# SIMPLE-BuildingSimulation/heat

Measured on AMD Instinct MI355X. Metric: surface-node-updates/sec, higher is better.
Workload: dtype f64

## Files before the change

heat_amd/csrc/batch.hip:

```cpp
#include <hip/hip_runtime.h>
#include <rccl/rccl.h>

#include <dlfcn.h>

#include <algorithm>
#include <cmath>
#include <cstdarg>
#include <cstdio>
#include <cstdlib>
#include <cstring>
#include <limits>
#include <mutex>
#include <numeric>
#include <string>
#include <vector>

#include "../../include/heat_amd.h"
#include "kernels.hpp"
#include "layout.hpp"
#include "hostpool.hpp"
#include "plan.hpp"

using namespace heat;

// ... 55 lines not shown
        r.CommDestroy = reinterpret_cast<decltype(r.CommDestroy)>(dlsym(h, "ncclCommDestroy"));
        r.AllGather = reinterpret_cast<decltype(r.AllGather)>(dlsym(h, "ncclAllGather"));
        r.AllReduce = reinterpret_cast<decltype(r.AllReduce)>(dlsym(h, "ncclAllReduce"));
        r.GetErrorString = reinterpret_cast<decltype(r.GetErrorString)>(dlsym(h, "ncclGetErrorString"));
        if (!r.GetUniqueId || !r.CommInitRank || !r.CommDestroy || !r.AllGather || !r.AllReduce || !r.GetErrorString) {
            st.err = "symbols missing";
            dlclose(h);
            return;
        }
        st.err.clear();
        r.handle = h;
    });
    return st.r.handle ? &st.r : nullptr;
}

#define RCCL_TRY(R, expr)                                                                             \
    do {                                                                                              \
        ncclResult_t e_ = (expr);                                                                     \
        if (e_ != ncclSuccess)                                                                        \
            return fail(HEAT_E_COMM, "%s failed: %s (%s:%d)", #expr, (R)->GetErrorString(e_), __FILE__, __LINE__); \
    } while (0)

template <typename T>
struct DevBuf {
    T *p = nullptr;
    size_t n = 0;
    ~DevBuf() { release(); }
    void release() {
        if (p) (void)hipFree(p);
        p = nullptr;
        n = 0;
    }
    hipError_t alloc(size_t count) {
        release();
        n = count;
        if (count == 0) return hipSuccess;
        return hipMalloc(reinterpret_cast<void **>(&p), count * sizeof(T));
    }
    hipError_t upload(const std::vector<T> &h) {
        hipError_t e = alloc(h.size());
        if (e != hipSuccess || h.empty()) return e;
        return hipMemcpy(p, h.data(), h.size() * sizeof(T), hipMemcpyHostToDevice);
    }
    hipError_t zeros(size_t count) {
        hipError_t e = alloc(count);
        if (e != hipSuccess || count == 0) return e;
        e = hipMemset(p, 0, count * sizeof(T));
        if (e != hipSuccess) return e;
        return hipStreamSynchronize(nullptr);
    }
};

static const int kFusedMinSubsteps = getenv("HEAT_AMD_FUSED_MIN") ? atoi(getenv("HEAT_AMD_FUSED_MIN")) : 2;

}

struct heat_batch {
    int device = 0;
    int n_cu = 256;
    hipStream_t stream = nullptr;
    bool own_stream = false;
    static constexpr int kSideStreams = 3;
    hipStream_t side[kSideStreams] = {nullptr, nullptr, nullptr};
    hipStream_t fused_stream = nullptr;
    hipEvent_t ev_fork = nullptr, ev_join[kSideStreams] = {nullptr, nullptr, nullptr};
    int n_ranks = 1, rank = 0;
    bool use_graph = false;

    int64_t n_surf = 0, n_zones = 0, n_state = 0, n_nodes = 0, n_cav = 0;
    double dt = 0;
    int64_t algorithmic_bytes = 0;
    int64_t class_counts[5] = {0, 0, 0, 0, 0};
    int64_t n_palette = 0;

    int64_t n_fused_surfaces = 0;
    int n_stream_tiles[kNumFast] = {};
    std::vector<FusedBlock> h_fblocks[kNumFast][4];
    DevBuf<FusedBlock> d_fblocks[kNumFast][4];
    std::vector<FusedBlock> h_team_blocks[kNumFast], h_team_blocks0[kNumFast];
    std::vector<FusedSuper> h_team_supers[kNumFast];
    DevBuf<FusedBlock> d_team_blocks[kNumFast];
    DevBuf<FusedSuper> d_team_supers[kNumFast];
    DevBuf<uint32_t> d_team_zinfo;
    DevBuf<unsigned long long> d_xbuf;
    int xbuf_teams = 0;
    uint32_t team_epoch = 0;
    bool any_teams = false;
    DevBuf<unsigned int> d_fqueue;
    DevBuf<int32_t> d_fzones, d_fzone_eoff;
    DevBuf<uint16_t> d_fslots;
    DevBuf<double> d_side_area;
    DevBuf<int16_t> d_side_lzone;
    std::vector<FastTile> h_tiles0[kNumFast];
    std::vector<FusedBlock> h_fblocks0[kNumFast][4];
    int n_stream_tiles0[kNumFast] = {};
    std::vector<int32_t> h_fzones;
    DevBuf<int32_t> d_zlist_stream;
    int n_touched_stream = 0;
    std::vector<int32_t> h_zone_block;
    DevBuf<int32_t> d_stream_zones;
    int n_stream_zones = 0;
    bool any_fused = false;
    hipEvent_t ev_fused = nullptr;
    hipEvent_t ev_staged = nullptr;
    bool staged = false;
    int n_fast_tiles[kNumFast] = {};
    DevBuf<FastTile> d_fast_tiles[kNumFast];
    std::vector<FastTile> h_tiles_cur[kNumFast];
    DevBuf<FastTile> d_ulist[2];
    int n_ulist[2] = {0, 0};
    int ulist_part[2][kStreamVariants][2] = {};
    bool capturing = false;
    bool host_zones_stale = false;
    unsigned int sweep_parity = 0;
    unsigned int fused_parity = 0;
    bool class_has_chunks[kNumFast] = {};
    bool in_ulist[2][kNumFast] = {};
    bool small_in_ulist[2] = {false, false};
    bool smallcav_in_ulist[2] = {false, false};
    DevBuf<unsigned long long> d_ucount;
    size_t ucount_stride = 0;
    int n_gen_tiles = 0;
    int n_small_tiles = 0;
    int n_small_plain_tiles = 0;
    int n_smallcav_stream_tiles = 0;
    int n_smallcav_stream_tiles0 = 0;
    std::vector<GeneralTile> h_gen_tiles0;
    std::vector<GeneralTile> h_gen_tiles_cur;
    size_t nm_count_base[kNumFast + 1] = {};
    DevBuf<GeneralTile> d_gen_tiles;
    int64_t gen_base = 0;
    int64_t node_slots = 0;

    DevBuf<double> d_T, d_V, d_U, d_alpha_f, d_alpha_b, d_mass, d_scratch;
    DevBuf<int32_t> d_cav_idx;
    DevBuf<int32_t> d_cavref;
    DevBuf<uint8_t> d_cls;
    DevBuf<double> d_pal;
    DevBuf<CavityDev> d_cavs;

    DevBuf<int32_t> d_meta;
// ... 563 lines not shown
    for (int c = 0; c < kNumFast; c++) {
        const int n_super = (int)b->h_team_supers[c].size();
        if (n_super == 0) continue;
        if (n_sub > 4095) return fail(HEAT_E_INVALID_ARG, "a march call of %d sub-timesteps: the team exchange tags 4095 at most", n_sub);
        static const int team_room_env = getenv("HEAT_AMD_TEAM_ROOM") ? atoi(getenv("HEAT_AMD_TEAM_ROOM")) : 0;
        TeamShape &ts = shape[c];
        ts.room = team_room_env > 0 ? team_room_env : b->n_cu * std::min(2, fused_team_blocks_per_cu(kFastM[c], kFastNM[c], b->na.pal_stride));
        ts.team_size = 2;
        for (const FusedSuper &su : b->h_team_supers[c]) ts.team_size = std::max(ts.team_size, (int)su.n_members);
        ts.n_teams = std::min(n_super, std::max(0, ts.room - ts.room / 8) / ts.team_size);
        if (ts.n_teams >= 1 && (n_super + ts.n_teams - 1) / ts.n_teams > 1023)
            return fail(HEAT_E_SIZE, "%d clusters for %d teams: the exchange tags 1023 rounds per launch at most", n_super, ts.n_teams);
        if (ts.n_teams < 1) return fail(HEAT_E_DEVICE, "the device holds %d workgroups of the team variant: not one team", ts.room);
    }
    return HEAT_OK;
}

int enqueue_fused(heat_batch *b, int n_sub, hipStream_t st, bool streamed_beside = false) {
    TeamShape team_shape[kNumFast];
    {
        const int rc = team_shapes(b, n_sub, team_shape);
        if (rc) return rc;
    }
    FusedArgs fa{};
    {
        static const bool zigzag_off = getenv("HEAT_AMD_NO_ZIGZAG") != nullptr;
        fa.reverse = (!zigzag_off && (b->fused_parity++ & 1)) ? 1 : 0;
    }
    fa.zones = b->d_fzones.p;
    fa.zone_eoff = b->d_fzone_eoff.p;
    fa.slots = b->d_fslots.p;
    fa.side_area = b->d_side_area.p;
    fa.side_lzone = b->d_side_lzone.p;
    fa.a0 = b->d_zone_a0.p;
    fa.b0 = b->d_zone_b0.p;
    fa.vol = b->d_zone_vol.p;
    fa.zone_T = b->d_zone_T.p;
    fa.dt = b->dt;
    fa.n_sub = n_sub;
    fa.gen_tiles = b->d_gen_tiles.p;
    fa.gen_base = b->gen_base;
    fa.small_iters = b->d_nomass_iters.p + b->nm_count_base[kNumFast];
    static const int reserve_env = getenv("HEAT_AMD_FUSED_RESERVE") ? atoi(getenv("HEAT_AMD_FUSED_RESERVE")) : -1;
    const bool beside_exchange = (b->comm != nullptr && b->shared_set && b->n_shared > 0) || reserve_env >= 0 || streamed_beside;
    double streamed_share = 0.0;
    if (streamed_beside) {
        double ns = 4.0 * kWave * (b->n_gen_tiles - (b->n_small_tiles - b->n_small_plain_tiles - b->n_smallcav_stream_tiles)), nf = 0.0;
        for (int c = 0; c < kNumFast; c++) {
            ns += (double)b->n_stream_tiles[c] * kFastM[c] * kWave;
            nf += (double)(b->n_fast_tiles[c] - b->n_stream_tiles[c]) * kFastM[c] * kWave;
        }
        streamed_share = ns / std::max(ns + nf, 1.0);
    }
    const int n_cu = b->n_cu;
    if (beside_exchange && b->d_fqueue.n == 0) HIP_TRY(b->d_fqueue.zeros(kNumFast * 4));
    for (int c = 0; c < kNumFast; c++)
        for (int g2 = 0; g2 < 4; g2++) {
            const int nb = (int)b->h_fblocks[c][g2].size();
            if (nb == 0) continue;
            fa.blocks = b->d_fblocks[c][g2].p;
            fa.n_blocks = nb;
            fa.queue = nullptr;
            int grid = nb;
            if (beside_exchange) {
                const int fw = (g2 & 1) ? 8 : 4;
                static const int room_env = getenv("HEAT_AMD_FUSED_ROOM") ? atoi(getenv("HEAT_AMD_FUSED_ROOM")) : 0;
                const int room = room_env > 0 ? room_env : n_cu * fused_blocks_per_cu(kFastM[c], kFastCAV[c], g2 >> 1, fw, b->na.pal_stride);
                const int reserve = reserve_env >= 0 ? reserve_env
                                                     : std::min(room / 2, std::max(fw == 4 ? 16 : 8, (int)(room * streamed_share)));
                if (nb > room - reserve) {
                    grid = std::max(1, room - reserve);
                    fa.queue = b->d_fqueue.p + c * 4 + g2;
                    HIP_TRY(hipMemsetAsync(fa.queue, 0, sizeof(unsigned int), st));
                }
            }
            static const bool trace = getenv("HEAT_AMD_TRACE") != nullptr;
            if (trace)
                fprintf(stderr, "heat_amd: fused launch%s: %d workgroups for %d blocks (class %d, list %d, %d sub-timesteps)\n",
                        fa.queue ? " on the work queue" : "", grid, nb, c, g2, n_sub);
            b->n_fused_launches++;
            const int nm_variant = kFastNM[c] ? ((b->class_has_chunks[c] && !(g2 >> 1) && !kFastCAV[c] && kFastM[c] <= 8) ? 2 : 1) : 0;
            HIP_TRY(launch_surfaces_fused(kFastM[c], nm_variant, kFastCAV[c], g2 >> 1, (g2 & 1) ? 8 : 4, grid, b->d_fast_tiles[c].p, b->n_fast_tiles[c],
                                          b->na, b->sa, b->d_weather.p, b->d_flags.p,
                                          b->d_nomass_iters.p + b->nm_count_base[c], fa, st));
        }
    for (int c = 0; c < kNumFast; c++) {
        const int n_super = (int)b->h_team_supers[c].size();
        if (n_super == 0) continue;
        const int team_size = team_shape[c].team_size, n_teams = team_shape[c].n_teams;
        if (b->xbuf_teams < n_teams) {
            HIP_TRY(b->d_xbuf.zeros((size_t)n_teams * 2 * kTeamZones * kTeamMax * 4));
            b->xbuf_teams = n_teams;
        }
        b->team_epoch++;
        if ((b->team_epoch & 1023u) == 0) {
            HIP_TRY(hipMemsetAsync(b->d_xbuf.p, 0, b->d_xbuf.n * sizeof(unsigned long long), st));
            b->team_epoch++;
        }
        fa.blocks = b->d_team_blocks[c].p;
        fa.n_blocks = (int)b->h_team_blocks[c].size();
        fa.queue = nullptr;
        fa.supers = b->d_team_supers[c].p;
        fa.n_super = n_super;
        fa.team_zinfo = b->d_team_zinfo.p;
        fa.xbuf = b->d_xbuf.p;
        fa.tag_base = (b->team_epoch & 1023u) << 22;
        fa.team_size = team_size;
        static const bool trace = getenv("HEAT_AMD_TRACE") != nullptr;
        if (trace)
            fprintf(stderr, "heat_amd: team launch: %d teams of %d workgroups for %d clusters (class %d, %d sub-timesteps)\n",
                    n_teams, team_size, n_super, c, n_sub);
        b->n_fused_launches++;
        HIP_TRY(launch_surfaces_fused(kFastM[c], kFastNM[c], 0, 2, 4, n_teams * team_size, b->d_fast_tiles[c].p, b->n_fast_tiles[c], b->na,
                                      b->sa, b->d_weather.p, b->d_flags.p, b->d_nomass_iters.p + b->nm_count_base[c], fa, st));
    }
    return HEAT_OK;
}

hipEvent_t next_event(heat_batch *b) {
    if (b->ev_used == b->ev_pool.size()) {
        hipEvent_t e;
        if (hipEventCreate(&e) != hipSuccess) return nullptr;
        b->ev_pool.push_back(e);
    }
    return b->ev_pool[b->ev_used++];
}

struct MarchGuard {
    heat_batch *b;
    double *saved_partial;
    bool forked = false, joined = false;
    explicit MarchGuard(heat_batch *b_) : b(b_), saved_partial(b_->partial_ptr) {}
    ~MarchGuard() {
        b->partial_ptr = saved_partial;
        if (forked && !joined && b->fused_stream) (void)hipStreamSynchronize(b->fused_stream);
    }
};
// ... 2102 lines not shown
```

heat_amd/csrc/kernels.hip:

```cpp
#include <hip/hip_runtime.h>

#include <algorithm>
#include <atomic>
#include <cstdlib>

#include "device_math.hpp"
#include "kernels.hpp"
#include "layout.hpp"

namespace heat {

__device__ __forceinline__ void eval_side(const SideConst &c, const StepWeather &w, double air_t, double rad_alt,
                                          double rad_out, double surf_t, double &hs, double &rad_t, int &bad) {
    const double natural = tarp_natural(air_t, surf_t, c.cos_eff, bad);
    if ((c.kind_n & 3) == KIND_OUTDOOR) {
        const bool windward = (c.kind_n & 4) ? true : ((c.nx * w.sin_wd + c.ny * w.cos_wd) > 0.0);
        const double wf = windward ? 1.0 : 0.5;
        hs = wf * (c.forced * w.sqrt_ws) + natural;
        rad_t = rad_out;
    } else {
        hs = natural;
        rad_t = rad_alt;
    }
}
// ... 353 lines not shown
        l.zvol[threadIdx.x] = fa.vol[z];
    }
    const int n_e = fa.zone_eoff[blk.first_zone + blk.n_zones] - e_first;
    for (int e = threadIdx.x; e < n_e; e += n_threads) l.slots[fa.slots[e_first + e]] = (unsigned short)e;
    __syncthreads();
}

struct FusedPre {
    int e_first, n_e, zoff, z, slot0;
    double zT, za0, zb0, zvol;
};
__device__ __forceinline__ void fused_pre_a(const FusedBlock &blk, const FusedArgs &fa, FusedPre &p) {
    p = FusedPre{0, 0, 0, 0, 0, 0.0, 0.0, 0.0, 0.0};
    const int nz = blk.n_zones;
    if (nz > 0) {
        p.e_first = fa.zone_eoff[blk.first_zone];
        p.n_e = fa.zone_eoff[blk.first_zone + nz];
        p.zoff = fa.zone_eoff[blk.first_zone + min((int)threadIdx.x, nz)];
        p.z = fa.zones[blk.first_zone + min((int)threadIdx.x, nz - 1)];
    }
}
__device__ __forceinline__ void fused_pre_b(const FusedBlock &blk, const FusedArgs &fa, FusedPre &p) {
    if (blk.n_zones > 0) {
        p.n_e -= p.e_first;
        p.zoff -= p.e_first;
        p.zT = fa.zone_T[p.z];
        p.za0 = fa.a0[p.z];
        p.zb0 = fa.b0[p.z];
        p.zvol = fa.vol[p.z];
        if (p.n_e > 0) p.slot0 = fa.slots[p.e_first + min((int)threadIdx.x, p.n_e - 1)];
    }
}
__device__ __forceinline__ void fused_block_init(const FusedBlock &blk, const FusedArgs &fa, const FusedLds &l, int n_threads,
                                                 const FusedPre &p) {
    if ((int)threadIdx.x <= blk.n_zones) l.zoff[threadIdx.x] = p.zoff;
    if ((int)threadIdx.x < blk.n_zones) {
        l.zT[threadIdx.x] = p.zT;
        l.za0[threadIdx.x] = p.za0;
        l.zb0[threadIdx.x] = p.zb0;
        l.zvol[threadIdx.x] = p.zvol;
    }
    if ((int)threadIdx.x < p.n_e) l.slots[p.slot0] = (unsigned short)threadIdx.x;
    for (int e = threadIdx.x + n_threads; e < p.n_e; e += n_threads) l.slots[fa.slots[p.e_first + e]] = (unsigned short)e;
    __syncthreads();
}

struct TeamCtx {
    int team, member, round, it;
    int *flags;
};
__device__ __forceinline__ unsigned long long team_granule(unsigned int data, unsigned int tag) {
    return ((unsigned long long)tag << 32) | data;
}
template <int TEAM>
__device__ __forceinline__ void fused_zone_phase(const FusedBlock &blk, const FusedArgs &fa, const FusedLds &l, int wib,
                                                 int n_waves, int lane, int &bad_all, const TeamCtx &tc_) {
    __syncthreads();
    auto team_area = [&](int j, unsigned int &mask, unsigned int &tag) -> unsigned long long * {
        const unsigned int info = fa.team_zinfo[blk.first_zone + j];
        mask = info >> 16;
        tag = fa.tag_base | ((unsigned int)tc_.round << 12) | (unsigned int)(tc_.it + 1);
        return fa.xbuf + ((((size_t)tc_.team * 2 + (tc_.it & 1)) * kTeamZones + (info & 0xffffu)) * kTeamMax) * 4;
    };
    auto publish = [&](int j, double a, double b) {
        unsigned int mask, tag;
        unsigned long long *g = team_area(j, mask, tag) + tc_.member * 4;
        const unsigned long long ab = (unsigned long long)__double_as_longlong(a), bb = (unsigned long long)__double_as_longlong(b);
        __hip_atomic_store(g + 0, team_granule((unsigned int)ab, tag), __ATOMIC_RELAXED, __HIP_MEMORY_SCOPE_AGENT);
        __hip_atomic_store(g + 1, team_granule((unsigned int)(ab >> 32), tag), __ATOMIC_RELAXED, __HIP_MEMORY_SCOPE_AGENT);
        __hip_atomic_store(g + 2, team_granule((unsigned int)bb, tag), __ATOMIC_RELAXED, __HIP_MEMORY_SCOPE_AGENT);
        __hip_atomic_store(g + 3, team_granule((unsigned int)(bb >> 32), tag), __ATOMIC_RELAXED, __HIP_MEMORY_SCOPE_AGENT);
    };
    auto gather = [&](int j, double &a, double &b) {
        unsigned int mask, tag;
        const unsigned long long *area = team_area(j, mask, tag);
        double sa = 0.0, sb = 0.0;
        for (int m = 0; m < kTeamMax; m++) {
            if (!((mask >> m) & 1u)) continue;
            double am = a, bm = b;
            if (m != tc_.member) {
                const unsigned long long *g = area + m * 4;
                unsigned long long g0 = 0, g1 = 0, g2 = 0, g3 = 0;
                bool got = false;
                for (int spin = 0; spin < (1 << 21); spin++) {
                    g0 = __hip_atomic_load(g + 0, __ATOMIC_RELAXED, __HIP_MEMORY_SCOPE_AGENT);
                    g1 = __hip_atomic_load(g + 1, __ATOMIC_RELAXED, __HIP_MEMORY_SCOPE_AGENT);
                    g2 = __hip_atomic_load(g + 2, __ATOMIC_RELAXED, __HIP_MEMORY_SCOPE_AGENT);
                    g3 = __hip_atomic_load(g + 3, __ATOMIC_RELAXED, __HIP_MEMORY_SCOPE_AGENT);
                    got = (unsigned int)(g0 >> 32) == tag && (unsigned int)(g1 >> 32) == tag &&
                          (unsigned int)(g2 >> 32) == tag && (unsigned int)(g3 >> 32) == tag;
                    if (got) break;
                    __builtin_amdgcn_s_sleep(4);
                }
                if (!got) atomicOr(tc_.flags, FLAG_EXCHANGE);
                am = __longlong_as_double((long long)((g0 & 0xffffffffull) | (g1 << 32)));
                bm = __longlong_as_double((long long)((g2 & 0xffffffffull) | (g3 << 32)));
            }
            sa += am;
            sb += bm;
        }
        a = sa;
        b = sb;
    };
    auto finish = [&](int j, double a, double b, double tc, double cz) {
        a += l.za0[j];
        b += l.zb0[j];
        double ft = tc;
        if (fabs(b) > 1e-9) ft = a / b + (tc - a / b) * exp(-b * fa.dt / cz);
        if (ft != ft) bad_all |= FLAG_NAN_ZONE;
        l.zT[j] = ft;
    };
    if (blk.n_zones <= n_waves) {
        if (wib < blk.n_zones) {
            const int j = wib;
            const int e0 = l.zoff[j], e1 = l.zoff[j + 1];
            const double tc = l.zT[j];
            const double cz = zone_mcp(l.zvol[j], tc);
            double a = 0.0, b = 0.0;
            for (int e = e0 + lane; e < e1; e += kWave) {
                const double2 ht = l.hT[e];
                a += ht.x * ht.y;
                b += ht.x;
            }
            a = wave_sum_f64(a);
            b = wave_sum_f64(b);
            if (lane == 0) {
                if constexpr (TEAM) {
                    publish(j, a, b);
                    gather(j, a, b);
                }
                finish(j, a, b, tc, cz);
            }
        }
    } else {
        const int row = lane >> 4, rl = lane & 15;
        const bool one_pass = blk.n_zones <= 4 * n_waves;
        (void)one_pass;
#pragma clang loop unroll(disable)
        for (int j0 = 0; j0 < blk.n_zones; j0 += 4 * n_waves) {
            const int j = j0 + 4 * wib + row;
            const bool on = j < blk.n_zones;
            const int jj = on ? j : 0;
            const int e0 = l.zoff[jj], e1 = on ? l.zoff[jj + 1] : e0;
            const double tc = l.zT[jj];
            const double cz = zone_mcp(l.zvol[jj], tc);
            double a = 0.0, b = 0.0;
            for (int e = e0 + rl; __any(e < e1); e += 16) {
                if (e < e1) {
                    const double2 ht = l.hT[e];
                    a += ht.x * ht.y;
                    b += ht.x;
                }
            }
            a = row_sum_f64(a);
            b = row_sum_f64(b);
            if constexpr (TEAM) {
                if (on && rl == 15) {
                    publish(j, a, b);
                    if (one_pass) {
                        gather(j, a, b);
                        finish(j, a, b, tc, cz);
                    } else {
                        l.zsa[j] = a;
                        l.zsb[j] = b;
                    }
                }
            } else {
                if (on && rl == 15) finish(j, a, b, tc, cz);
            }
        }
        if constexpr (TEAM) {
            if (!one_pass) {
#pragma clang loop unroll(disable)
                for (int j0 = 0; j0 < blk.n_zones; j0 += 4 * n_waves) {
                    const int j = j0 + 4 * wib + row;
                    if (j < blk.n_zones && rl == 15) {
                        const double tc = l.zT[j];
                        const double cz = zone_mcp(l.zvol[j], tc);
                        double a = l.zsa[j], b = l.zsb[j];
                        gather(j, a, b);
                        finish(j, a, b, tc, cz);
                    }
                }
            }
        }
    }
    __syncthreads();
}

#pragma clang fp contract(off)
__device__ void fused_small_wave(const FusedBlock &blk, const FusedArgs &fa, const FusedLds &l, int lanes_per_side,
                                 int wib, int n_waves, int lane, const NodeArrays &na, const SideArrays &sd,
                                 const StepWeather *__restrict__ weather, int *__restrict__ flags) {
    const int tile_index = blk.first_small + (wib - blk.n_tiles);
    const GeneralTile tile = fa.gen_tiles[tile_index];
    weather = site_weather(weather, sd, tile.surf_base);
    const bool active = lane < tile.G;
    const int d = tile.surf_base + (active ? lane : 0);
    const int S = sd.S;
    const SideConst cf = sd.sc[d];
    const SideConst cb = sd.sc[S + d];
    const SideDyn df = sd.dyn[d];
    const SideDyn db = sd.dyn[S + d];
    const int nn = cf.kind_n >> 16;
    const int lz_f = fa.side_lzone[d], lz_b = fa.side_lzone[S + d];
    const double area = fa.side_area[d];
    Nodes4 T{0.0, 0.0, 0.0, 0.0};
    double Us[kSmallNodes], sol[kSmallNodes];
    int cav[kSmallNodes];
    CavityDev cv[kSmallNodes - 1];
    small_load<1>(tile, active ? lane : 0, na, fa.gen_base, df, db, nn, T, Us, sol, cav, cv);
    fused_block_init(blk, fa, l, n_waves * kWave);
    int bad_all = 0;
    unsigned int iters = 0;
    SideOut of{0.0, 0.0}, ob{0.0, 0.0};
    auto btemp = [&](const SideConst &c, int lz, const StepWeather &w) -> double {
        const int kind = c.kind_n & 3;
        if (kind == KIND_SPACE) return l.zT[lz];
        if (kind == KIND_AMBIENT) return c.ambient;
        return w.t_out;
    };
#pragma clang loop unroll(disable)
    for (int it = 0; it < fa.n_sub; it++) {
        const StepWeather w = weather[it];
        int bad = 0;
        small_step<1>(cf, cb, df, db, sd.hs_fix, d, S, w, btemp(cf, lz_f, w), btemp(cb, lz_b, w), nn, T, Us, sol, cav,
                      cv, bad, iters, of, ob);
        if (active) {
            bad_all |= bad;
            const double Tl = T.last(nn);
            if ((cf.kind_n & 3) == KIND_SPACE) l.hT[l.slots[wib * kWave + lane]] = make_double2(of.hs * area, T.a);
            if ((cb.kind_n & 3) == KIND_SPACE) l.hT[l.slots[lanes_per_side + wib * kWave + lane]] = make_double2(ob.hs * area, Tl);
        }
        fused_zone_phase<0>(blk, fa, l, wib, n_waves, lane, bad_all, TeamCtx{0, 0, 0, 0, nullptr});
    }
    if ((int)threadIdx.x < blk.n_zones) fa.zone_T[fa.zones[blk.first_zone + threadIdx.x]] = l.zT[threadIdx.x];
    if (active) {
        double *Tg = na.T + tile.node_base + lane;
#pragma unroll
        for (int j = 0; j < kSmallNodes; j++) if (j < nn) Tg[(int64_t)j * kWave] = T.get(j);
        sd.out[d] = of;
        sd.out[S + d] = ob;
        if (fa.small_iters) fa.small_iters[(int64_t)tile_index * kWave + lane] += iters;
    }
    if (bad_all) report_failure(flags, bad_all, (unsigned int)d);
}
#pragma clang fp contract(fast)

#ifdef HEAT_STAMPS
constexpr int kStampsPerBlock = 8;
__device__ unsigned long long g_stamps[65536 * kStampsPerBlock];
#define HEAT_STAMP(k, real)                                                                                   \
    do {                                                                                                      \
        if constexpr (FUSED) {                                                                                \
            if (threadIdx.x == 0 && (counter_index >> 2) < 65536)                                             \
                g_stamps[(counter_index >> 2) * kStampsPerBlock + (k)] =                                      \
                    (real) ? __builtin_amdgcn_s_memrealtime() : __builtin_amdgcn_s_memtime();                 \
        }                                                                                                     \
    } while (0)
#else
#define HEAT_STAMP(k, real) do { } while (0)
#endif
#ifdef HEAT_STREAM_STAMPS
#ifndef HEAT_STAMPS
constexpr int kStampsPerBlock = 8;
__device__ unsigned long long g_stamps[65536 * kStampsPerBlock];
#endif
#define HEAT_SSTAMP(k, drain)                                                                                  \
    do {                                                                                                       \
        if constexpr (!FUSED && PAL) {                                                                         \
            if (drain) asm volatile("s_waitcnt vmcnt(0) lgkmcnt(0)" ::: "memory");                             \
            if (lane == 0 && counter_index < 32768)                                                            \
                g_stamps[(counter_index + (M == 16 ? 32768 : 0)) * kStampsPerBlock + (k)] = __builtin_amdgcn_s_memtime(); \
        }                                                                                                      \
    } while (0)
#else
#define HEAT_SSTAMP(k, drain) do { } while (0)
#endif

template <int M, int NM, int PAL, int CAV, int FUSED, int SMALL = 0>
__device__ __forceinline__ void fast_tile_march(const FastTile tile, int counter_index, bool nm_on, int lane, int wib,
                                                double *s_pal, double *s_V, double *s_pos, const FusedLds &fl, const FusedBlock &blk,
                                                int blk_waves, int n_it, int step0, const NodeArrays &na,
                                                const SideArrays &sd, const StepWeather *__restrict__ weather,
                                                const double *__restrict__ zone_T, int *__restrict__ flags,
                                                unsigned long long *__restrict__ nomass_iters, const FusedArgs &fa,
                                                bool write_out = true, const TeamCtx team = TeamCtx{0, 0, 0, 0, nullptr}) {
    constexpr int kLanes = (FUSED ? FUSED : 4) * kWave;
    constexpr bool kVinLds = FUSED && fused_v_in_lds(M, NM, FUSED, SMALL);
    HEAT_STAMP(4, true);
    HEAT_STAMP(0, false);
    HEAT_SSTAMP(0, false);
    double2 *const s_hT = fl.hT;
    double *const s_zT = fl.zT;
    (void)s_hT; (void)s_zT; (void)s_V; (void)s_pos; (void)nm_on; (void)blk; (void)blk_waves; (void)counter_index;
    FusedPre pre;
    (void)pre;
    if constexpr (FUSED) fused_pre_a(blk, fa, pre);
    const bool mixed = PAL && (tile.k & kTileMixedBit) != 0;
    constexpr bool kChunks = NM == 2 && PAL;
    const bool chunky = kChunks && (tile.k & kTileChunkyBit) != 0;
    const int k = tile.k & 0xff;
    const bool full = (tile.k & 0x100) != 0;
    const int G = tile.G;
    const int Lk = mixed ? k : (kWave / k) * k;
    int g = (int)(((float)lane + 0.5f) * (1.0f / (float)k));
    int seg = lane - g * k;
    bool is_last = (seg == k - 1);
    const bool in_layout = lane < Lk;
    if (mixed) {
        const unsigned int e = reinterpret_cast<const unsigned short *>(na.cls + tile.node_base + (int64_t)M * Lk)[in_layout ? lane : 0];
        g = (int)(e & 63u);
        seg = (int)((e >> 6) & 63u);
        is_last = (e & (unsigned int)kLaneLastBit) != 0;
// ... 108 lines not shown
            const double2 t = pT[jp * Lk + ll];
            const double2 v = pV[jp * Lk + ll];
            const double2 u = pU[jp * Lk + ll];
            T[2 * jp] = t.x; T[2 * jp + 1] = t.y;
            V[2 * jp] = v.x; V[2 * jp + 1] = v.y;
            U[2 * jp] = u.x; U[2 * jp + 1] = u.y;
        }
    }
    HEAT_STAMP(7, false);
    if constexpr (FUSED) fused_block_init(blk, fa, fl, blk_waves * kWave, pre);

    const int first_lane = lane - seg;
    const int nn = kind_n_mine >> 16;
    const int jl = full ? (M - 1) : (nn - 1 - (mixed ? seg : k - 1) * M);

    auto pick_last = [&](const double (&x)[M]) {
        double r = x[M - 1];
        if (!full) {
#pragma unroll
            for (int j = 0; j < M - 1; j++) r = (j == jl) ? +x[j] : +r;
        }
        return r;
    };

    const bool wave_quirk = __any((is_last && (kind_n_mine & 3) == KIND_AMBIENT && my_back) ||
                                  (single && ((kind_n_mine >> 4) & 3) == KIND_AMBIENT));
    double zt_mine = 0.0, zt_b2 = 0.0;
    (void)zt_mine; (void)zt_b2;
    if constexpr (!FUSED) {
        zt_mine = zone_T[c_load.zone];
        if constexpr (kSingleLane) zt_b2 = zone_T[cb2.zone];
    }

    auto Vat = [&](int j) -> double {
        if constexpr (kVinLds) return s_V[j * kLanes + threadIdx.x];
        else return V[j];
    };
    auto V_last = [&]() {
        double r = Vat(M - 1);
        if (!full) {
#pragma unroll
            for (int j = 0; j < M - 1; j++) r = (j == jl) ? Vat(j) : r;
        }
        return r;
    };

    int bad_all = 0;
    unsigned int nm_passes = 0;
    double o_hs = 0.0, o_flow = 0.0, o2_hs = 0.0, o2_flow = 0.0;
    StepWeather w_next = weather[step0];

    HEAT_STAMP(1, false);
    HEAT_SSTAMP(1, true);
    SideConst c_cur = c_load;
    SideDyn dy_cur = dy_load;
#pragma clang loop unroll(disable)
    for (int it = 0; it < n_it; it++) {
    const StepWeather w = w_next;
    if constexpr (FUSED) w_next = weather[min(it + 1, n_it - 1)];
    const SideConst c = c_cur;
    const SideDyn dy = dy_cur;
    auto btemp = [&](const SideConst &cc, int lz, double zt) -> double {
        const int kind = cc.kind_n & 3;
        if (kind == KIND_SPACE) {
            if constexpr (FUSED) return s_zT[lz];
            else return zt;
        }
        if (kind == KIND_AMBIENT) return cc.ambient;
        return w.t_out;
    };

    int bad = 0;
    auto prepare = [&](const SideConst &cc, const SideDyn &dd, bool back, int rec, int lz, double zt, double &air_t,
                       double &rad_t, double &forced, bool &use_front_T) {
        const int kind = cc.kind_n & 3;
        air_t = btemp(cc, lz, zt);
        rad_t = air_t;
        use_front_T = false;
        forced = 0.0;
        if (kind == KIND_OUTDOOR) {
            const bool windward = (cc.kind_n & 4) ? true : ((cc.nx * w.sin_wd + cc.ny * w.cos_wd) > 0.0);
            forced = (windward ? 1.0 : 0.5) * (cc.forced * w.sqrt_ws);
            rad_t = dd.rad_t;
        } else if (back && kind == KIND_AMBIENT) {
            const int fkind = (cc.kind_n >> 4) & 3;
            if (fkind == KIND_SPACE) {
                if constexpr (FUSED) rad_t = s_zT[peer_lz];
                else rad_t = zt;
            } else if (fkind == KIND_AMBIENT) {
                rad_t = cc.forced;
            } else {
                rad_t = w.t_out;
            }
            use_front_T = true;
        }
        (void)rec;
    };
    auto conv = [&](double air_t, double forced, double nat_pos, double nat_neg, int rec, double surf_t) {
        double hs = forced + tarp_natural_coef(air_t, surf_t, nat_pos, nat_neg, bad);
        if (hs != hs) bad |= FLAG_NAN_HS;
        if (sd.hs_fix != nullptr) {
            const double fix = sd.hs_fix[rec];
            if (fix == fix) hs = fix;
        }
        return hs;
    };
// ... 245 lines not shown
    if constexpr (!FUSED) {
        if (active) {
            double2 *pT = reinterpret_cast<double2 *>(na.T + tile.node_base);
#pragma unroll
            for (int jp = 0; jp < M / 2; jp++) pT[jp * Lk + lane] = make_double2(T[2 * jp], T[2 * jp + 1]);
        }
    }

    const double T0n = wave_quirk ? shfl_f64(T[0], first_lane) : T[0];
    const double Tln = pick_last(T);
    const double Tnn = Tln;
    {
        const double surf_t = (my_back && !my_useF) ? Tnn : T0n;
        const double hs = conv(my_air, my_forced, c.cos_eff, c.alpha, sidx, surf_t);
        const double face_t = my_back ? Tln : T[0];
        o_hs = hs;
        o_flow = (face_t - my_air) * hs;
        if constexpr (!FUSED) {
            if (active && (is_first || is_last) && (kind_n_mine & 3) == KIND_SPACE) {
                ZoneContrib z;
                z.ha = hs * c.forced;
                z.t_face = face_t;
                sd.zc[__double_as_longlong(s_pos[threadIdx.x])] = z;
            }
        }
        if constexpr (FUSED) {
            if (active && (is_first || is_last) && (c.kind_n & 3) == KIND_SPACE)
                s_hT[fl.slots[(my_back ? kLanes : 0) + wib * kWave + lane]] = make_double2(hs * my_area, face_t);
        }
    }
    if (single) {
        const double hs = conv(b_air, b_forced, b_cos, b_neg, S + d, b_useF ? T0n : Tnn);
        o2_hs = hs;
        o2_flow = (Tln - b_air) * hs;
        if constexpr (!FUSED) {
            if (active) put_zone_contrib(sd, cb2, hs, Tln);
        } else {
            if (active && (cb2.kind_n & 3) == KIND_SPACE)
                s_hT[fl.slots[kLanes + wib * kWave + lane]] = make_double2(hs * my_area, Tln);
        }
    } else if (!(is_first || is_last)) {
        bad = 0;
    }
    bad_all |= bad;

    if constexpr (FUSED) {
        int sidx_next = sidx;
        asm volatile("" : "+v"(sidx_next));
        c_cur = sd.sc[sidx_next];
        dy_cur = sd.dyn[sidx_next];
        if constexpr (SMALL == 2) {
            TeamCtx tcx = team;
            tcx.it = it;
            fused_zone_phase<1>(blk, fa, fl, wib, blk_waves, lane, bad_all, tcx);
        } else {
            fused_zone_phase<0>(blk, fa, fl, wib, blk_waves, lane, bad_all, team);
        }
    }
    }
    HEAT_STAMP(2, false);
    HEAT_SSTAMP(2, false);

    if constexpr (FUSED) {
        if (active) {
            double2 *pT = reinterpret_cast<double2 *>(na.T + tile.node_base);
#pragma unroll
            for (int jp = 0; jp < M / 2; jp++) pT[jp * Lk + lane] = make_double2(T[2 * jp], T[2 * jp + 1]);
        }
        if (threadIdx.x < blk.n_zones) fa.zone_T[fa.zones[blk.first_zone + threadIdx.x]] = s_zT[threadIdx.x];
    }
    if (write_out && active && (is_first || is_last)) {
        SideOut o;
        o.hs = o_hs;
        o.flow = o_flow;
        sd.out[sidx] = o;
    }
    if (write_out && single && active) {
        SideOut o;
        o.hs = o2_hs;
        o.flow = o2_flow;
        sd.out[S + d] = o;
    }
    if (active && bad_all) report_failure(flags, bad_all, (unsigned int)d);
#ifdef HEAT_STAMPS
    asm volatile("s_waitcnt vmcnt(0)" ::: "memory");
#endif
    HEAT_STAMP(3, false);
    HEAT_SSTAMP(3, true);
    HEAT_STAMP(5, true);
    if constexpr (NM) {
        unsigned int tot = nm_passes;
#pragma unroll
        for (int o = kWave / 2; o > 0; o >>= 1) tot += __shfl_down(tot, o, kWave);
        if (lane == 0 && tot) nomass_iters[counter_index] += tot;
    }
}

template <int M, int NM, int PAL, int CAV, int FUSED, int SMALL = 0>
__global__ void __launch_bounds__(FUSED ? 64 * FUSED : 256, (FUSED || (M == 16 && !CAV)) ? 2 : 1)
k_surfaces_fast(const FastTile *__restrict__ tiles, int n_tiles, NodeArrays na, SideArrays sd,
                const StepWeather *__restrict__ weather, const int *__restrict__ step_ptr, int step_fixed,
                const double *__restrict__ zone_T, int *__restrict__ flags,
                unsigned long long *__restrict__ nomass_iters, FusedArgs fa) {
    static_assert(!FUSED || (PAL && !(CAV && M == 16)),
                  "the cluster-resident march exists for palette classes; with gas cavities for 4 or 8 nodes per lane");
    constexpr int kMaxW = FUSED ? FUSED : 4;
    constexpr int kLanes = kMaxW * kWave;
    extern __shared__ double s_dyn[];
    __shared__ double s_pos_static[FUSED ? 2 : kLanes];
    double *const s_pal = s_dyn;
    constexpr bool kVinLds = FUSED && fused_v_in_lds(M, NM, FUSED, SMALL);
    double *const s_V = s_dyn + kLanes * na.pal_stride;
    FusedLds fl;
// ... 22 lines not shown
    int sb = 0, n_teams = 1;
    if constexpr (kTeam) {
        team.team = (int)blockIdx.x / fa.team_size;
        team.member = (int)blockIdx.x % fa.team_size;
        n_teams = (int)gridDim.x / fa.team_size;
        sb = team.team;
    }
    for (int wave = wave0; FUSED ? (kTeam ? (sb < fa.n_super) : (bi < fa.n_blocks)) : (wave < n_tiles); wave += n_waves) {
    if constexpr (FUSED) {
        if constexpr (kTeam) {
            const FusedSuper su = fa.supers[fa.reverse ? fa.n_super - 1 - sb : sb];
            if (team.member >= su.n_members) {
                sb += n_teams;
                team.round++;
                continue;
            }
            bi = su.first_block + team.member;
        }
        blk = fa.blocks[(!kTeam && fa.reverse) ? fa.n_blocks - 1 - bi : bi];
        blk_waves = blk.n_tiles + (SMALL == 1 ? blk.n_small : 0);
        const bool looping = kTeam || fa.queue != nullptr;
        if (wib >= blk_waves) {
            if (!looping) return;
            for (int q = 0; q < kFusedBarriersAtInit; q++) __syncthreads();
            for (int it = 0; it < fa.n_sub; it++)
                for (int q = 0; q < kFusedBarriersPerSubstep; q++) __syncthreads();
            goto next_block;
        }
        if constexpr (SMALL == 1) {
            if (wib >= blk.n_tiles) {
                fused_small_wave(blk, fa, fl, kLanes, wib, blk_waves, lane, na, sd, weather, flags);
                if (!looping) return;
                goto next_block;
            }
        }
        wave = blk.first_tile + wib;
    }
    {
    const int tix = (!FUSED && fa.reverse) ? n_tiles - 1 - wave : wave;
    const FastTile tl = tiles[tix];
    fast_tile_march<M, NM, PAL, CAV, FUSED, SMALL>(tl, tix, true, lane, wib, s_pal, s_V, s_pos_static, fl, blk, blk_waves, n_it, step0, na,
                                                   sd, site_weather(weather, sd, tl.surf_base), zone_T, flags, nomass_iters, fa,
                                                   write_out, team);
    }
next_block:
    if constexpr (FUSED) {
        if constexpr (kTeam) {
            __syncthreads();
            sb += n_teams;
            team.round++;
        } else {
            if (fa.queue == nullptr) break;
            __syncthreads();
            if (threadIdx.x == 0) s_next_block = (int)(gridDim.x + atomicAdd(fa.queue, 1u));
            __syncthreads();
            bi = s_next_block;
        }
    }
    }
}

constexpr int kTileKindShift = 9;
constexpr int kTileNmBit = 1 << 11;
enum { kStreamWide = 0, kStreamLight = 1, kStreamChunks = 2, kStreamCav = 3 };
template <int VARIANT>
__global__ void __launch_bounds__(256, VARIANT == kStreamLight ? 3 : 2)
k_surfaces_stream(const FastTile *__restrict__ tiles, int n_tiles, NodeArrays na, int64_t gen_base, SideArrays sd,
                  const StepWeather *__restrict__ weather, const int *__restrict__ step_ptr, int step_fixed,
                  const double *__restrict__ zone_T, int *__restrict__ flags,
                  unsigned long long *__restrict__ nomass_iters, int reverse) {
    extern __shared__ double s_pal[];
    __shared__ double s_pos[4 * kWave];
    const int lane = threadIdx.x & (kWave - 1);
    const int wib = threadIdx.x >> 6;
    const int wave0 = blockIdx.x * (blockDim.x >> 6) + wib;
    const int n_waves = gridDim.x * (blockDim.x >> 6);
    const int step0 = (step_fixed >= 0) ? step_fixed : *step_ptr;
    const bool write_out = step_fixed >= 0 || step0 == step_ptr[1];
    const FusedLds fl{};
    const FusedBlock blk{0, 0, 0, 0, 0, 0};
    const FusedArgs fa{};
    if (wave0 >= n_tiles) return;
    constexpr int kNm = VARIANT == kStreamChunks ? 2 : 1;
    const int last = n_tiles - 1;
    FastTile tile_next = tiles[__builtin_amdgcn_readfirstlane(reverse ? last - wave0 : wave0)];
    int site_next = sd.site ? tile_site(sd, tile_next.surf_base) : 0;
    for (int wv = wave0; wv < n_tiles; wv += n_waves) {
        const int w = __builtin_amdgcn_readfirstlane(reverse ? last - wv : wv);
        FastTile tile = tile_next;
        const StepWeather *const wt = weather + (int64_t)site_next * sd.wstride;
        const int wn = min(wv + n_waves, last);
        tile_next = tiles[__builtin_amdgcn_readfirstlane(reverse ? last - wn : wn)];
        const int kind = (tile.k >> kTileKindShift) & 3;
        const bool nm = (tile.k & kTileNmBit) != 0;
        tile.k = (int16_t)(tile.k & (0x1ff | kTileMixedBit | kTileChunkyBit));
        if constexpr (VARIANT == kStreamWide) {
            fast_tile_march<16, 0, 1, 0, 0>(tile, w, false, lane, wib, s_pal, nullptr, s_pos, fl, blk, 0, 1, step0, na, sd, wt,
                                            zone_T, flags, nomass_iters, fa, write_out);
        } else {
            constexpr int kCav = VARIANT == kStreamCav ? 1 : 0;
            switch (kind) {
            case 1:
                fast_tile_march<8, kNm, 1, kCav, 0>(tile, w, nm, lane, wib, s_pal, nullptr, s_pos, fl, blk, 0, 1, step0, na, sd, wt,
                                                    zone_T, flags, nomass_iters, fa, write_out);
                break;
            case 0:
                fast_tile_march<4, kNm, 1, kCav, 0>(tile, w, nm, lane, wib, s_pal, nullptr, s_pos, fl, blk, 0, 1, step0, na, sd, wt,
// ... 1814 lines not shown
```

heat_amd/csrc/layout.hpp:

```cpp
#pragma once
#include <stdint.h>

namespace heat {

constexpr int kWave = 64;
constexpr double kSigma = 5.670374419e-8;
constexpr double kMassThreshold = 1e-5;

enum : int { KIND_SPACE = 0, KIND_AMBIENT = 1, KIND_OUTDOOR = 2 };

enum ShadeRow : int { SH_NX, SH_NY, SH_NZ, SH_UX, SH_UY, SH_UZ, SH_VX, SH_VY, SH_VZ, SH_W, SH_H, SH_OD, SH_OG, SH_PD, SH_PG, SH_ND,
                      SH_NG, SH_FD, SH_FG, kShadeRows };

enum : int { FLAG_NAN_HS = 1, FLAG_NAN_NOMASS = 2, FLAG_NAN_ZONE = 4, FLAG_UNREACHABLE = 8,
              FLAG_EXCHANGE = 16 };

struct FastTile {
    int64_t node_base;
    int32_t surf_base;
    int16_t k;
    int16_t G;
};
constexpr int kTileMixedBit = 1 << 12;
constexpr int kTileChunkyBit = 1 << 13;
// ... 59 lines not shown

struct NodeArrays {
    double *T;
    const double *V;
    const double *U;
    const uint8_t *cls;
    const double *pal;
    const int32_t *cavref;
    const struct CavityDev *cavs;
    const double *alpha_f;
    const double *alpha_b;
    const int32_t *cav;
    const double *mass;
    int32_t pal_stride;
    int32_t pal_ubase;
};

struct CavityDev {
    double thickness, height, angle, eout, ein;
    int32_t gas, pad;
};

struct StepWeather {
    double t_out;
    double sqrt_ws;
    double sin_wd, cos_wd;
};

constexpr int kFusedMaxWaves = 8;
constexpr int kFusedMaxZones = 32;
constexpr int kFusedMaxEntries = 1024;
struct FusedBlock {
    int32_t first_tile;
    int32_t n_tiles;
    int32_t first_zone;
    int32_t n_zones;
    int32_t first_small;
    int32_t n_small;
};
struct FusedArgs {
    const FusedBlock *blocks;
    const int32_t *zones;
    const int32_t *zone_eoff;
    const uint16_t *slots;
    const double *side_area;
    const int16_t *side_lzone;
    const double *a0, *b0, *vol;
    double *zone_T;
    double dt;
    int32_t n_sub;
    int32_t pad;
    unsigned int *queue;
    int32_t n_blocks;
    int32_t pad2;
    const GeneralTile *gen_tiles;
    int64_t gen_base;
    unsigned long long *small_iters;
    const struct FusedSuper *supers;
    const uint32_t *team_zinfo;
    unsigned long long *xbuf;
    int32_t n_super;
    uint32_t tag_base;
    int32_t team_size;
    int32_t reverse;
};

constexpr int kTeamMax = 8;
constexpr int kTeamZones = 256;
struct FusedSuper {
    int32_t first_block;
    int32_t n_members;
};

struct ZoneEntry {
    uint32_t t_index;
    uint32_t hs_index;
    double area;
};

}
```

Measured before the change: 514.6 billion.

## Use persistent work-queue fused launches for long runs and prioritize zone-phase waves

When the number of sub-timesteps reaches a threshold, fused launches are capped at the occupancy room, and workgroups pull the remaining blocks from an atomic queue, with no reserve unless running beside an exchange. A host-tracked queue base replaces the per-launch memset of the queue counter: the counter keeps growing across launches and each launch subtracts its starting offset. Waves doing zone-phase work also raise their scheduling priority with s_setprio so the serial zone reduction finishes sooner. Optional timestamp instrumentation is added but compiled out by default. The risks are atomic contention on the queue, load imbalance when grids are capped, and priority changes that may starve other waves.

```diff
diff --git a/heat_amd/csrc/batch.hip b/heat_amd/csrc/batch.hip
--- a/heat_amd/csrc/batch.hip
+++ b/heat_amd/csrc/batch.hip
@@ -131,6 +131,7 @@
 };
 
 static const int kFusedMinSubsteps = getenv("HEAT_AMD_FUSED_MIN") ? atoi(getenv("HEAT_AMD_FUSED_MIN")) : 2;
+constexpr int kFusedQueueMinSubsteps = 12;
 
 }
 
@@ -166,6 +167,7 @@
     uint32_t team_epoch = 0;
     bool any_teams = false;
     DevBuf<unsigned int> d_fqueue;
+    unsigned int fqueue_base[kNumFast * 4] = {};
     DevBuf<int32_t> d_fzones, d_fzone_eoff;
     DevBuf<uint16_t> d_fslots;
     DevBuf<double> d_side_area;
@@ -835,8 +837,11 @@
         }
         streamed_share = ns / std::max(ns + nf, 1.0);
     }
+    static const int persist_env = getenv("HEAT_AMD_FUSED_PERSIST") ? atoi(getenv("HEAT_AMD_FUSED_PERSIST")) : -1;
+    const int persist_min = persist_env >= 0 ? persist_env : kFusedQueueMinSubsteps;
+    const bool persist = persist_min > 0 && n_sub >= persist_min;
     const int n_cu = b->n_cu;
-    if (beside_exchange && b->d_fqueue.n == 0) HIP_TRY(b->d_fqueue.zeros(kNumFast * 4));
+    if (b->d_fqueue.n == 0) HIP_TRY(b->d_fqueue.zeros(kNumFast * 4));
     for (int c = 0; c < kNumFast; c++)
         for (int g2 = 0; g2 < 4; g2++) {
             const int nb = (int)b->h_fblocks[c][g2].size();
@@ -845,16 +850,16 @@
             fa.n_blocks = nb;
             fa.queue = nullptr;
             int grid = nb;
-            if (beside_exchange) {
+            if (beside_exchange || persist) {
                 const int fw = (g2 & 1) ? 8 : 4;
                 static const int room_env = getenv("HEAT_AMD_FUSED_ROOM") ? atoi(getenv("HEAT_AMD_FUSED_ROOM")) : 0;
                 const int room = room_env > 0 ? room_env : n_cu * fused_blocks_per_cu(kFastM[c], kFastCAV[c], g2 >> 1, fw, b->na.pal_stride);
-                const int reserve = reserve_env >= 0 ? reserve_env
+                const int reserve = !beside_exchange ? 0 : reserve_env >= 0 ? reserve_env
                                                      : std::min(room / 2, std::max(fw == 4 ? 16 : 8, (int)(room * streamed_share)));
                 if (nb > room - reserve) {
                     grid = std::max(1, room - reserve);
                     fa.queue = b->d_fqueue.p + c * 4 + g2;
-                    HIP_TRY(hipMemsetAsync(fa.queue, 0, sizeof(unsigned int), st));
+                    fa.queue_base = b->fqueue_base[c * 4 + g2];
                 }
             }
             static const bool trace = getenv("HEAT_AMD_TRACE") != nullptr;
@@ -866,6 +871,7 @@
             HIP_TRY(launch_surfaces_fused(kFastM[c], nm_variant, kFastCAV[c], g2 >> 1, (g2 & 1) ? 8 : 4, grid, b->d_fast_tiles[c].p, b->n_fast_tiles[c],
                                           b->na, b->sa, b->d_weather.p, b->d_flags.p,
                                           b->d_nomass_iters.p + b->nm_count_base[c], fa, st));
+            if (fa.queue) b->fqueue_base[c * 4 + g2] += (unsigned int)nb;
         }
     for (int c = 0; c < kNumFast; c++) {
         const int n_super = (int)b->h_team_supers[c].size();
diff --git a/heat_amd/csrc/kernels.hip b/heat_amd/csrc/kernels.hip
--- a/heat_amd/csrc/kernels.hip
+++ b/heat_amd/csrc/kernels.hip
@@ -429,10 +429,23 @@
 __device__ __forceinline__ unsigned long long team_granule(unsigned int data, unsigned int tag) {
     return ((unsigned long long)tag << 32) | data;
 }
+constexpr int kZonePrio = 2;
+__device__ __forceinline__ void zone_prio_raise(bool lead) {
+    if (__builtin_amdgcn_readfirstlane((int)lead)) __builtin_amdgcn_s_setprio(kZonePrio);
+}
+__device__ __forceinline__ void zone_prio_drop() { __builtin_amdgcn_s_setprio(0); }
 template <int TEAM>
 __device__ __forceinline__ void fused_zone_phase(const FusedBlock &blk, const FusedArgs &fa, const FusedLds &l, int wib,
-                                                 int n_waves, int lane, int &bad_all, const TeamCtx &tc_) {
+                                                 int n_waves, int lane, int &bad_all, const TeamCtx &tc_,
+                                                 unsigned long long *clk = nullptr) {
+#ifdef HEAT_STAMPS
+    const unsigned long long t_in = __builtin_amdgcn_s_memtime();
+#endif
     __syncthreads();
+#ifdef HEAT_STAMPS
+    const unsigned long long t_open = __builtin_amdgcn_s_memtime();
+#endif
+    const int wib_u = __builtin_amdgcn_readfirstlane(wib), nz_u = __builtin_amdgcn_readfirstlane(blk.n_zones);
     auto team_area = [&](int j, unsigned int &mask, unsigned int &tag) -> unsigned long long * {
         const unsigned int info = fa.team_zinfo[blk.first_zone + j];
         mask = info >> 16;
@@ -488,6 +501,7 @@
         l.zT[j] = ft;
     };
     if (blk.n_zones <= n_waves) {
+        if constexpr (!TEAM) zone_prio_raise(wib_u < nz_u);
         if (wib < blk.n_zones) {
             const int j = wib;
             const int e0 = l.zoff[j], e1 = l.zoff[j + 1];
@@ -509,6 +523,7 @@
                 finish(j, a, b, tc, cz);
             }
         }
+        if constexpr (!TEAM) zone_prio_drop();
     } else {
         const int row = lane >> 4, rl = lane & 15;
         const bool one_pass = blk.n_zones <= 4 * n_waves;
@@ -517,6 +532,7 @@
         for (int j0 = 0; j0 < blk.n_zones; j0 += 4 * n_waves) {
             const int j = j0 + 4 * wib + row;
             const bool on = j < blk.n_zones;
+            if constexpr (!TEAM) zone_prio_raise(j0 + 4 * wib_u < nz_u);
             const int jj = on ? j : 0;
             const int e0 = l.zoff[jj], e1 = on ? l.zoff[jj + 1] : e0;
             const double tc = l.zT[jj];
@@ -544,6 +560,7 @@
                 }
             } else {
                 if (on && rl == 15) finish(j, a, b, tc, cz);
+                zone_prio_drop();
             }
         }
         if constexpr (TEAM) {
@@ -562,6 +579,12 @@
             }
         }
     }
+#ifdef HEAT_STAMPS
+    if (clk) {
+        clk[0] += t_open - t_in;
+        clk[1] += __builtin_amdgcn_s_memtime() - t_open;
+    }
+#endif
     __syncthreads();
 }
 
@@ -625,8 +648,15 @@
 #pragma clang fp contract(fast)
 
 #ifdef HEAT_STAMPS
-constexpr int kStampsPerBlock = 8;
+constexpr int kStampsPerBlock = 16;
 __device__ unsigned long long g_stamps[65536 * kStampsPerBlock];
+#define HEAT_STAMP_VALUE(k, v)                                                                                \
+    do {                                                                                                      \
+        if constexpr (FUSED) {                                                                                \
+            if (threadIdx.x == 0 && (counter_index >> 2) < 65536)                                             \
+                g_stamps[(counter_index >> 2) * kStampsPerBlock + (k)] = (v);                                 \
+        }                                                                                                     \
+    } while (0)
 #define HEAT_STAMP(k, real)                                                                                   \
     do {                                                                                                      \
         if constexpr (FUSED) {                                                                                \
@@ -637,6 +667,7 @@
     } while (0)
 #else
 #define HEAT_STAMP(k, real) do { } while (0)
+#define HEAT_STAMP_VALUE(k, v) do { } while (0)
 #endif
 #ifdef HEAT_STREAM_STAMPS
 #ifndef HEAT_STAMPS
@@ -851,6 +882,8 @@
 
     HEAT_STAMP(1, false);
     HEAT_SSTAMP(1, true);
+    unsigned long long chain_clk[2] = {0ull, 0ull};
+    (void)chain_clk;
     SideConst c_cur = c_load;
     SideDyn dy_cur = dy_load;
 #pragma clang loop unroll(disable)
@@ -1202,13 +1235,15 @@
         if constexpr (SMALL == 2) {
             TeamCtx tcx = team;
             tcx.it = it;
-            fused_zone_phase<1>(blk, fa, fl, wib, blk_waves, lane, bad_all, tcx);
+            fused_zone_phase<1>(blk, fa, fl, wib, blk_waves, lane, bad_all, tcx, chain_clk);
         } else {
-            fused_zone_phase<0>(blk, fa, fl, wib, blk_waves, lane, bad_all, team);
+            fused_zone_phase<0>(blk, fa, fl, wib, blk_waves, lane, bad_all, team, chain_clk);
         }
     }
     }
     HEAT_STAMP(2, false);
+    HEAT_STAMP_VALUE(8, chain_clk[0]);
+    HEAT_STAMP_VALUE(9, chain_clk[1]);
     HEAT_SSTAMP(2, false);
 
     if constexpr (FUSED) {
@@ -1337,7 +1372,7 @@
         } else {
             if (fa.queue == nullptr) break;
             __syncthreads();
-            if (threadIdx.x == 0) s_next_block = (int)(gridDim.x + atomicAdd(fa.queue, 1u));
+            if (threadIdx.x == 0) s_next_block = (int)(gridDim.x + (atomicAdd(fa.queue, 1u) - fa.queue_base));
             __syncthreads();
             bi = s_next_block;
         }
diff --git a/heat_amd/csrc/layout.hpp b/heat_amd/csrc/layout.hpp
--- a/heat_amd/csrc/layout.hpp
+++ b/heat_amd/csrc/layout.hpp
@@ -135,7 +135,7 @@
     int32_t pad;
     unsigned int *queue;
     int32_t n_blocks;
-    int32_t pad2;
+    uint32_t queue_base;
     const GeneralTile *gen_tiles;
     int64_t gen_base;
     unsigned long long *small_iters;
```

Measured after the change: 530.7 billion (median of 6 runs). 3.1% higher.
